# haan6/fm-for-online-recommendation

Measured on AMD Instinct MI355X. Metric: samples/sec online-FM (Criteo-39-field, k=16) FTRL-proximal, higher is better.
Workload: dtype f32

## Files before the change

fm-for-online-recommendation_amd/csrc/fmx_common.h:

```cpp
#pragma once
#include <hip/hip_runtime.h>
#include <hip/hip_ext.h>

#include <cstdarg>
#include <cstdio>
#include <cstdlib>
#include <cstring>
#include <atomic>
#include <mutex>

#include "fmx.h"

#pragma clang fp contract(off)

namespace fmxd {
extern thread_local char g_err[512];
int fail(int code, const char *fmt, ...);
int check_launch(const char *what);

struct Tune {
  int wpb_fwd = 4, wpb_upd = 2;
  int sort_e = 0;
  int inline_fixup = 1;
  int online_persistent = 1;
// ... 202 lines not shown
    s = s + xor_lane_f4<M>(s, lane);
    ss = ss + xor_lane_f4<M>(ss, lane);
    fo += xor_lane_f<M>(fo, lane);
  }
}
template <int LPR>
__device__ __forceinline__ void fm_field_sums(float4 &s, float4 &ss, float &fo, int lane, int groups = WAVE) {
  fm_sums_level<1, LPR>(s, ss, fo, lane, groups);
  fm_sums_level<2, LPR>(s, ss, fo, lane, groups);
  fm_sums_level<4, LPR>(s, ss, fo, lane, groups);
  fm_sums_level<8, LPR>(s, ss, fo, lane, groups);
  fm_sums_level<16, LPR>(s, ss, fo, lane, groups);
  fm_sums_level<32, LPR>(s, ss, fo, lane, groups);
}
template <int LPR>
__device__ __forceinline__ float4 fm_bi(float4 s, float4 ss, float &sbi) {
  const float4 bi = 0.5f * (s * s - ss);
  sbi = (bi.x + bi.y) + (bi.z + bi.w);
#pragma unroll
  for (int m = 1; m < LPR; m <<= 1) sbi += __shfl_xor(sbi, m);
  return bi;
}
template <int LPR>
__device__ __forceinline__ float4 fm_bi_dpp(float4 s, float4 ss, float &sbi) {
  const float4 bi = 0.5f * (s * s - ss);
  sbi = (bi.x + bi.y) + (bi.z + bi.w);
  if (LPR > 1) sbi += xor_lane_f<1>(sbi, 0);
  if (LPR > 2) sbi += xor_lane_f<2>(sbi, 0);
  if (LPR > 4) sbi += xor_lane_f<4>(sbi, 0);
  if (LPR > 8) sbi += xor_lane_f<8>(sbi, 0);
  return bi;
}

__device__ float block_sum(const float *src, int n, int ld, float *sm) {
  constexpr int U = 16;
  const int tid = threadIdx.x, nt = blockDim.x < 128 ? blockDim.x : 128;
  float acc = 0.f;
  if (tid >= nt) {
    __syncthreads();
    for (int w = nt >> 1; w > 0; w >>= 1) __syncthreads();
    const float r = sm[0];
    __syncthreads();
    return r;
  }
  if (ld == 1) {
    const int n4 = n >> 2;
    const float4 *src4 = reinterpret_cast<const float4 *>(src);
    for (int i0 = tid; i0 < n4; i0 += U * nt) {
      float4 v[U];
#pragma unroll
      for (int u = 0; u < U; ++u) {
        const int i = i0 + u * nt;
        v[u] = src4[i < n4 ? i : 0];
      }
#pragma unroll
      for (int u = 0; u < U; ++u) {
        const bool in = i0 + u * nt < n4;
        acc += in ? (v[u].x + v[u].y) + (v[u].z + v[u].w) : 0.f;
      }
    }
    for (int i = (n4 << 2) + tid; i < n; i += nt) acc += src[i];
  } else {
    constexpr int V = 4;
    const int n4 = n >> 2;
    for (int i0 = tid; i0 < n4; i0 += V * nt) {
      float4 v[V];
#pragma unroll
      for (int u = 0; u < V; ++u) {
        const int i = i0 + u * nt;
        const float *p = src + (size_t)(4 * (i < n4 ? i : 0)) * ld;
        v[u] = float4{p[0], p[ld], p[2 * (size_t)ld], p[3 * (size_t)ld]};
      }
#pragma unroll
      for (int u = 0; u < V; ++u) {
        const bool in = i0 + u * nt < n4;
        acc += in ? (v[u].x + v[u].y) + (v[u].z + v[u].w) : 0.f;
      }
    }
    for (int i = (n4 << 2) + tid; i < n; i += nt) acc += src[(size_t)i * ld];
  }
  sm[tid] = acc;
  __syncthreads();
  for (int w = nt >> 1; w > 0; w >>= 1) {
    if (tid < w) sm[tid] += sm[tid + w];
    __syncthreads();
  }
  const float r = sm[0];
  __syncthreads();
  return r;
}

__device__ __forceinline__ float ld_sc1(const float *p) {
  return __hip_atomic_load(p, __ATOMIC_RELAXED, __HIP_MEMORY_SCOPE_AGENT);
}
__device__ __forceinline__ float4 ld_sc1_4(const float *p) { return {ld_sc1(p), ld_sc1(p + 1), ld_sc1(p + 2), ld_sc1(p + 3)}; }

__device__ __forceinline__ void st16(float *p, float4 v) {
  typedef float f4v __attribute__((ext_vector_type(4)));
  __builtin_nontemporal_store(f4v{v.x, v.y, v.z, v.w}, reinterpret_cast<f4v *>(p));
}
__device__ __forceinline__ void st4(float *p, float v) { __builtin_nontemporal_store(v, p); }

struct RowRegs {
  float4 v;
  float4 z, n;
  float4 fo;
};

template <int LAYOUT, int RULE>
__device__ __forceinline__ RowRegs load_row(const float *rp, int q, int kp, int zoff) {
  RowRegs r;
  r.v = *reinterpret_cast<const float4 *>(rp + 4 * q);
  r.z = splat(0.f);
  r.n = splat(0.f);
  r.fo = splat(0.f);
  if (LAYOUT == FMX_LAYOUT_WEIGHTS) {
    r.fo.x = rp[kp];
  } else {
    if (LAYOUT == FMX_LAYOUT_FTRL || RULE == FMX_RULE_ADAM) r.z = *reinterpret_cast<const float4 *>(rp + zoff + 4 * q);
    r.n = *reinterpret_cast<const float4 *>(rp + zoff + kp + 4 * q);
    r.fo = *reinterpret_cast<const float4 *>(rp + kp);
  }
  return r;
}

template <int LAYOUT, int RULE>
__device__ __forceinline__ void update_row(float *rp, int q, int kp, int zoff, RowRegs r, float4 cV, float4 cA, float cw,
                                           const fmx_hyper_t &h) {
// ... 142 lines not shown
```

fm-for-online-recommendation_amd/csrc/fmx_kernels.hip:

```cpp

#include <type_traits>

#include "fmx_common.h"

namespace fmxd {

thread_local char g_err[512] = "";

int fail(int code, const char *fmt, ...) {
  va_list ap;
  va_start(ap, fmt);
  vsnprintf(g_err, sizeof(g_err), fmt, ap);
  va_end(ap);
  return code;
}

int check_launch(const char *what) {
  hipError_t e = hipGetLastError();
  if (e != hipSuccess) return fail(FMX_ERR_LAUNCH, "%s: %s", what, hipGetErrorString(e));
  return FMX_OK;
}

}

// ... 356 lines not shown
      bce_loss_dz(a.loss_kind, z, y_early, a.inv_b, loss, dz);
      if (a.out.loss) a.out.loss[(size_t)b * a.ld1] = loss;
      if (a.out.dz) a.out.dz[(size_t)b * a.ld1] = dz;
    }
  }
}

struct UpdArgs {
  float *rows;
  const int64_t *foff;
  float *bias;
  const uint32_t *sorted;
  float *parts;
  int32_t *meta;
  const float *xv;
  const float *S;
  const float *dz_first;
  const float *dz_bi;
  const float *gbi;
  const float *loss_b;
  float *loss_out;
  int32_t *step_counter;
  fmx_hyper_t h;
  int32_t B, F, Bp, bbits, kp, stride, zoff;
  int32_t ldS, ld1;
  int32_t ldG;
  const int32_t *cols;
  const int32_t *fcols;
  int32_t Fx;
  float *red;
  uint32_t seq;
  int32_t *error;
  float inv_b;
};

constexpr int LEAD_NONE = 0, LEAD_CLOSES = 1, LEAD_THROUGH = 2;

constexpr int RED_SLICE = 4096;
__host__ __device__ inline int red_slices(int B) { return (B + RED_SLICE - 1) / RED_SLICE; }

template <int LAYOUT, int RULE>
__device__ __forceinline__ void apply_bias_and_loss(const UpdArgs &a, float db, float ls) {
  constexpr bool MOM = LAYOUT == FMX_LAYOUT_MOMENTS;
  float b0 = a.bias[0], b1 = LAYOUT != FMX_LAYOUT_WEIGHTS ? a.bias[1] : 0.f, b2 = MOM ? a.bias[2] : 0.f;
  bias_step<LAYOUT, RULE>(b0, b1, b2, db, a.h);
  st4(a.bias, b0);
  if (LAYOUT == FMX_LAYOUT_FTRL || (MOM && RULE == FMX_RULE_ADAM)) st4(a.bias + 1, b1);
  if (MOM) st4(a.bias + 2, b2);
  if (a.loss_b && a.loss_out) {
    int i = 0;
    if (a.step_counter) {
      i = *a.step_counter;
      *a.step_counter = i + 1;
    }
    a.loss_out[i] = ls * a.inv_b;
  }
}

template <int LAYOUT, int RULE>
__device__ void finish_bias_and_loss(const UpdArgs &a, int R, bool poll) {
  __shared__ float part[2 * 16];
  const int t = threadIdx.x;
  bool failed = false;
  if (t < R) {
    const v4f *src = reinterpret_cast<const v4f *>(a.red) + t;
    v4f g = {0.f, 0.f, 0.f, 0.f};
    if (poll) {
      for (int spin = 0;; ++spin) {
        asm volatile("global_load_dwordx4 %0, %1, off sc1\n\ts_waitcnt vmcnt(0)" : "=v"(g) : "v"(src) : "memory");
        if (__float_as_uint(g.z) == a.seq) break;
        if (spin >= (1 << 20)) {
          failed = true;
          break;
        }
        __builtin_amdgcn_s_sleep(1);
      }
    } else {
      g = *src;
    }
    part[2 * t] = g.x;
    part[2 * t + 1] = g.y;
  }
  if (failed && a.error) *a.error = 2;
  __syncthreads();
  if (t == 0) {
    float db = 0.f, ls = 0.f;
    for (int r = 0; r < R; ++r) {
      db += part[2 * r];
      ls += part[2 * r + 1];
    }
    apply_bias_and_loss<LAYOUT, RULE>(a, db, ls);
  }
}

template <int LAYOUT, int RULE, bool INL>
__device__ void bias_and_loss(const UpdArgs &a, int r) {
  __shared__ float sm[256];
  const int R = red_slices(a.B);
  const int first = r * RED_SLICE, n = (a.B - first) < RED_SLICE ? (a.B - first) : RED_SLICE;
  const float db = block_sum(a.dz_first + (size_t)first * a.ld1, n, a.ld1, sm);
  float ls = 0.f;
  if (a.loss_b && a.loss_out) ls = block_sum(a.loss_b + (size_t)first * a.ld1, n, a.ld1, sm);
  if (R == 1) {
    if (threadIdx.x == 0) apply_bias_and_loss<LAYOUT, RULE>(a, db, ls);
    return;
  }
  if (threadIdx.x == 0) st_sc1_4(a.red + 4 * r, float4{db, ls, __uint_as_float(a.seq), 0.f});
  if (INL && r == 0) finish_bias_and_loss<LAYOUT, RULE>(a, R, true);
}

__device__ __forceinline__ void store_part(float *rec, int q, int kp, float4 cV, float4 cA, float cw) {
  *reinterpret_cast<float4 *>(rec + 4 * q) = cV;
  *reinterpret_cast<float4 *>(rec + kp + 4 * q) = cA;
  if (q == 0) rec[2 * kp] = cw;
}

template <bool VEC> struct CoefA;
template <> struct CoefA<true> {
  float4 v;
  __device__ __forceinline__ void zero() { v = splat(0.f); }
  __device__ __forceinline__ void add(const CoefA &o) { v = v + o.v; }
  __device__ __forceinline__ float4 vec() const { return v; }
  __device__ __forceinline__ CoefA up(int d) const { return {shfl_up4(v, d)}; }
};
template <> struct CoefA<false> {
  float v;
  __device__ __forceinline__ void zero() { v = 0.f; }
  __device__ __forceinline__ void add(const CoefA &o) { v += o.v; }
  __device__ __forceinline__ float4 vec() const { return splat(v); }
  __device__ __forceinline__ CoefA up(int d) const { return {__shfl_up(v, d)}; }
};

#ifdef FMX_STAMPS
__device__ unsigned long long g_upd_stamps[8192 * 6];
#define FMX_STAMP(slot_, dep_)                                                                                      \
  do {                                                                                                              \
    unsigned long long t_;                                                                                          \
    asm volatile("s_memrealtime %0\n\ts_waitcnt lgkmcnt(0)" : "=s"(t_) : "v"(dep_) : "memory");                      \
    if (lane == 0 && gt < 8192) g_upd_stamps[(size_t)gt * 6 + (slot_)] = t_;                                         \
  } while (0)
#else
#define FMX_STAMP(slot_, dep_) do {} while (0)
#endif

template <int LPR, int LAYOUT, int RULE, bool HAS_GBI, bool INL, bool OCC = false>
__device__ __forceinline__ void update_body(const UpdArgs &a, const int blk) {
  constexpr int SLOTS = WAVE / LPR;
  constexpr int EPG = LPR;
  constexpr int REC = 2 * LPR * 4 + 4;
  constexpr bool PREFETCH_ROWS = EPG <= 4;
  using CA = CoefA<HAS_GBI>;
  const int n_red = red_slices(a.B);
  if (blk < n_red) {
    bias_and_loss<LAYOUT, RULE, INL>(a, blk);
    return;
  }
  const int lane = threadIdx.x & 63;
  const int slot = lane / LPR, q = lane % LPR;
  const int kp = LPR * 4;
  const int tiles_per_field = a.Bp >> 6;
  const int gt = (blk - n_red) * (blockDim.x >> 6) + (threadIdx.x >> 6);
  if (gt >= a.F * tiles_per_field) return;
  const int f = gt / tiles_per_field;
  const int base = (gt - f * tiles_per_field) << 6;
  const uint32_t *sf = a.sorted + (size_t)f * a.Bp;
  const int bbits = a.bbits;
  const uint32_t bmask = (1u << bbits) - 1u;
  const int e0 = base + slot * EPG;
  FMX_STAMP(0, lane);

  uint32_t c[EPG];
  if constexpr (EPG % 4 == 0) {
#pragma unroll
    for (int j = 0; j < EPG; j += 4) {
      const uint4 t = *reinterpret_cast<const uint4 *>(sf + e0 + j);
      c[j] = t.x;
      c[j + 1] = t.y;
      c[j + 2] = t.z;
      c[j + 3] = t.w;
    }
  } else {
#pragma unroll
    for (int j = 0; j < EPG; ++j) c[j] = sf[e0 + j];
  }
  const uint32_t kprev = (e0 == 0 ? SENT : sf[e0 - 1]) >> bbits;
  const uint32_t knext = (e0 + EPG < a.Bp ? sf[e0 + EPG] : SENT) >> bbits;
  const uint32_t tile_prevkey = (base == 0 ? SENT : sf[base - 1]) >> bbits;
// ... 26 lines not shown
    if (INL)
      row_in = load_row<LAYOUT, RULE>(a.rows + (row0 + ((slot == 0 && run_comes_in) ? tile_prevkey : 0u)) * (size_t)a.stride, q, kp, a.zoff);
  };
  const bool tile_open_early = INL && __shfl((int)(val[EPG - 1] && k[EPG - 1] == knext), WAVE - 1) != 0;
  float4 cV[EPG];
  CA cA[EPG];
  float cw[EPG];
  {
    const bool has_x = a.xv != nullptr;
    const float *xsrc = has_x ? a.xv : a.dz_first;
    const int fld = (has_x && a.cols) ? a.cols[f] : f;
    const int col = (has_x && a.fcols) ? a.fcols[fld] : fld;
    int efld = 0;
    if constexpr (OCC) efld = a.cols ? a.cols[f] : f;
    float4 S4[EPG], G4[EPG];
    float xl[EPG], dzf[EPG], dzbl[EPG];
    uint32_t bj[EPG];
#pragma unroll
    for (int j = 0; j < EPG; ++j) bj[j] = val[j] ? (c[j] & bmask) : 0u;
    const bool sep_dzbi = a.dz_bi != nullptr && a.dz_bi != a.dz_first;
#pragma unroll
    for (int j = 0; j < EPG; ++j) {
      xl[j] = 1.f;
      dzbl[j] = 0.f;
    }
    if (has_x) {
#pragma unroll
      for (int j = 0; j < EPG; ++j) xl[j] = xsrc[(size_t)bj[j] * a.Fx + col];
    }
    if (sep_dzbi) {
#pragma unroll
      for (int j = 0; j < EPG; ++j) dzbl[j] = a.dz_bi[(size_t)bj[j] * a.ld1];
    }
#pragma unroll
    for (int j = 0; j < EPG; ++j) {
      const uint32_t b = bj[j];
      if constexpr (OCC) S4[j] = *reinterpret_cast<const float4 *>(a.gbi + (size_t)b * a.ldG + (size_t)efld * kp + 4 * q);
      else S4[j] = *reinterpret_cast<const float4 *>(a.S + (size_t)b * a.ldS + 4 * q);
      dzf[j] = a.dz_first[(size_t)b * a.ld1];
      if constexpr (HAS_GBI) G4[j] = *reinterpret_cast<const float4 *>(a.gbi + (size_t)b * a.ldG + 4 * q);
      else G4[j] = splat(0.f);
    }
    if (!tile_open_early) request_rows();
#pragma unroll
    for (int j = 0; j < EPG; ++j) {
      const float x = xl[j];
      const float dzb = a.dz_bi ? (sep_dzbi ? dzbl[j] : dzf[j]) : 0.f;
      const float w1 = x * dzf[j];
      float4 v;
      CA ca;
      if constexpr (OCC) {
        v = S4[j];
        ca.zero();
      } else if constexpr (HAS_GBI) {
        const float4 G = splat(dzb) + G4[j];
        const float4 xG = x * G;
        v = xG * S4[j];
        ca.v = x * xG;
      } else {
        const float xG = x * dzb;
        v = xG * S4[j];
        ca.v = x * xG;
      }
      cV[j] = splat(0.f);
      cA[j].zero();
      cw[j] = 0.f;
      if (val[j]) {
        cV[j] = v;
        cA[j] = ca;
        cw[j] = w1;
      }
    }
  }

  float4 tV = splat(0.f);
  CA tA;
// ... 137 lines not shown
      }
      __builtin_amdgcn_s_sleep(1);
    }
  }
  if (failed || m == 0 || m > t) {
    if (lane == 0 && a.error) *a.error = 2;
    return;
  }
  const size_t gh = (size_t)gt - m;
  float4 aV = splat(0.f), aA = splat(0.f);
  float aw = 0.f;
  for (int j = slot; j <= m; j += SLOTS) {
    if (j == m) {
      aV = aV + ownV;
      aA = aA + ownA;
      aw += ownw;
    } else {
      const float *rec = j == 0 ? a.parts + (gh * 2 + 1) * REC : a.parts + (gh + j) * 2 * REC;
      aV = aV + ld_sc1_4(rec + 4 * q);
      aA = aA + ld_sc1_4(rec + kp + 4 * q);
      aw += ld_sc1(rec + 2 * kp);
    }
  }
#pragma unroll
  for (int mm = LPR; mm < WAVE; mm <<= 1) {
    aV = aV + shfl_xor4(aV, mm);
    aA = aA + shfl_xor4(aA, mm);
    aw += __shfl_xor(aw, mm);
  }
  if (lane < LPR) update_row<LAYOUT, RULE>(rp, q, kp, a.zoff, r, aV, aA, aw, a.h);
  FMX_STAMP(4, lane);
}

template <int LPR, int LAYOUT, int RULE, bool HAS_GBI, bool INL>
__global__ __launch_bounds__(256) void k_fm_update(UpdArgs a) {
  __builtin_amdgcn_s_setprio(3);
  update_body<LPR, LAYOUT, RULE, HAS_GBI, INL>(a, blockIdx.x);
}

template <int LPR, int LAYOUT, int RULE, bool INL>
__global__ __launch_bounds__(256) void k_fm_update_occ(UpdArgs a) {
  __builtin_amdgcn_s_setprio(3);
  update_body<LPR, LAYOUT, RULE, false, INL, true>(a, blockIdx.x);
}

template <int LPR, int LAYOUT, int RULE, bool HAS_GBI>
__global__ __launch_bounds__(256) void k_fm_update_rider(UpdArgs a, MlpReduceArgs r, int n_update_blocks, int rider_blocks_per_layer) {
  __builtin_amdgcn_s_setprio(3);
  if ((int)blockIdx.x >= n_update_blocks) {
    const int rb = (int)blockIdx.x - n_update_blocks;
    mlp_reduce_block(r, rb / rider_blocks_per_layer, rb % rider_blocks_per_layer, rider_blocks_per_layer);
    return;
  }
  update_body<LPR, LAYOUT, RULE, HAS_GBI, true>(a, blockIdx.x);
}

struct OnlineArgs {
  float *rows;
  const int64_t *foff;
  float *bias;
  const int32_t *idx;
  const float *xv;
  const float *y;
  uint8_t *pred;
  float *loss;
  int32_t *error;
  fmx_hyper_t h;
  int32_t N, F, stride, zoff, loss_kind;
};

// ... 703 lines not shown
  snprintf(msg, sizeof(msg), "%s", g_err);
  return fail(rc, "%s: %s", who, msg);
}
Tune &tune() {
  static Tune t = [] {
    Tune x;
    if (const char *e = getenv("FMX_WPB_FWD")) x.wpb_fwd = atoi(e);
    if (const char *e = getenv("FMX_WPB_UPD")) x.wpb_upd = atoi(e);
    if (const char *e = getenv("FMX_SORT_E")) x.sort_e = atoi(e);
    if (const char *e = getenv("FMX_SORT_AHEAD")) x.sort_ahead = atoi(e);
    if (const char *e = getenv("FMX_ONLINE_PERSISTENT")) x.online_persistent = atoi(e);
    if (const char *e = getenv("FMX_INLINE_FIXUP")) x.inline_fixup = atoi(e);
    if (const char *e = getenv("FMX_SORT_CHUNKED")) x.sort_chunked = atoi(e);
    if (const char *e = getenv("FMX_MLP_CHAIN")) x.mlp_chain = atoi(e);
    auto ok = [](int v) { return v == 1 || v == 2 || v == 4; };
    if (!ok(x.wpb_fwd)) x.wpb_fwd = 4;
    if (!ok(x.wpb_upd)) x.wpb_upd = 2;
    return x;
  }();
  return t;
}
}
namespace {

constexpr int SORT_AHEAD_MAX = 16;

struct Workspace {
  uint32_t *sorted;
  size_t sorted_stride;
  uint32_t *runs;
  int32_t *meta;
  int32_t *counter;
  float *parts;
  size_t bytes;
};



Workspace carve(const fmx_table_t *t, int B, void *base) {
  const size_t F = (size_t)n_sort_fields(t), Bp = (size_t)fmx_sorted_width(B), tiles = Bp >> 6;
  const size_t rec = 2 * (size_t)t->kp + 4;
  const size_t o_sorted1 = align_up(F * Bp * 4, 256);
  const size_t o_runs = 2 * SORT_AHEAD_MAX * o_sorted1;
  const size_t o_meta = o_runs + (Bp >= 2 * SORT_CHUNK ? SORT_AHEAD_MAX * o_sorted1 : 0);
  const size_t o_counter = o_meta + align_up(F * tiles * 2 * 4, 256);
  const size_t o_parts = o_counter + 256;
  Workspace w;
  char *p = static_cast<char *>(base);
  w.sorted = reinterpret_cast<uint32_t *>(p);
  w.sorted_stride = o_sorted1 / 4;
  w.runs = reinterpret_cast<uint32_t *>(p + o_runs);
  w.meta = reinterpret_cast<int32_t *>(p + o_meta);
  w.counter = reinterpret_cast<int32_t *>(p + o_counter);
  w.parts = reinterpret_cast<float *>(p + o_parts);
  w.bytes = o_parts + align_up(F * tiles * 2 * rec * 4, 256);
  return w;
}

int check_workspace(const fmx_table_t *t, int B, const void *workspace, int64_t workspace_bytes, const char *who) {
  if (!workspace) return fail(FMX_ERR_ARG, "%s: null workspace", who);
  if (!aligned16(workspace)) return fail(FMX_ERR_ALIGN, "%s: workspace must be 16-byte aligned", who);
  const int64_t need = (int64_t)carve(t, B, nullptr).bytes;
  if (workspace_bytes < need)
    return fail(FMX_ERR_SHAPE, "%s: workspace of %lld bytes, %lld needed for B = %d and %d sort fields (fmx_workspace_bytes)", who,
                (long long)workspace_bytes, (long long)need, B, n_sort_fields(t));
  return FMX_OK;
}

struct Side {
  hipStream_t stream = nullptr;
  hipStream_t main = nullptr;
  hipEvent_t fork = nullptr, sorted[2] = {nullptr, nullptr}, consumed[2] = {nullptr, nullptr};
  hipEvent_t user_fork = nullptr, user_join = nullptr;
};

Side *side_for_current_device() {
  static std::mutex mu;
  static Side sides[64];
  int dev = 0;
  if (hipGetDevice(&dev) != hipSuccess || dev < 0 || dev >= 64) return nullptr;
  std::lock_guard<std::mutex> lock(mu);
  Side &sd = sides[dev];
  if (!sd.stream) {
    int lo = 0, hi = 0;
    (void)hipDeviceGetStreamPriorityRange(&lo, &hi);
    if (hipStreamCreateWithPriority(&sd.stream, hipStreamNonBlocking, lo) != hipSuccess) return nullptr;
    if (hipStreamCreateWithPriority(&sd.main, hipStreamNonBlocking, hi) != hipSuccess) return nullptr;
    bool ok = hipEventCreateWithFlags(&sd.fork, hipEventDisableTiming) == hipSuccess &&
// ... 4 lines not shown
           hipEventCreateWithFlags(&sd.consumed[i], hipEventDisableTiming) == hipSuccess;
    }
    if (!ok) return nullptr;
  }
  return &sd;
}

constexpr int OVERLAP_MIN_BATCH = 512;

template <int LPR, int NPASS, bool MAPPED = false>
void launch_forward_np(const FwdArgs &a, int layout, hipStream_t st) {
  const int wpb = tune().wpb_fwd;
  const dim3 grid((a.B + wpb - 1) / wpb), block(64 * wpb);
  if (layout == FMX_LAYOUT_FTRL) hipLaunchKernelGGL((k_fm_forward<LPR, FMX_LAYOUT_FTRL, NPASS, MAPPED>), grid, block, 0, st, a);
  else hipLaunchKernelGGL((k_fm_forward<LPR, FMX_LAYOUT_WEIGHTS, NPASS, MAPPED>), grid, block, 0, st, a);
}

template <int LPR>
void launch_forward(const FwdArgs &a, int layout, hipStream_t st) {
  const int slots = WAVE / LPR;
  const int np = (a.F + slots - 1) / slots;
  if (a.fcols || a.fbase)
    launch_forward_np<LPR, 0, true>(a, layout, st);
  else if (!with_one_of<1, 2, 3, 4>(np, [&](auto NP) { launch_forward_np<LPR, NP>(a, layout, st); }))
    launch_forward_np<LPR, 0>(a, layout, st);
}

bool is_capturing(hipStream_t st) {
  if (!st) return false;
  hipStreamCaptureStatus cs = hipStreamCaptureStatusNone;
  return hipStreamIsCapturing(st, &cs) == hipSuccess && cs != hipStreamCaptureStatusNone;
}

template <int LPR, bool HAS_GBI, bool INL>
void launch_update(const UpdArgs &a, int rule, hipStream_t st) {
  const int tiles = a.F * (a.Bp >> 6);
  const int wpb = tune().wpb_upd;
  const dim3 grid((tiles + wpb - 1) / wpb + red_slices(a.B)), block(64 * wpb);
  with_rule(rule, [&](auto LAYOUT, auto RULE) { hipLaunchKernelGGL((k_fm_update<LPR, LAYOUT, RULE, HAS_GBI, INL>), grid, block, 0, st, a); });
}

template <int LPR>
void launch_update_rider(const UpdArgs &a, int rule, const MlpReduceArgs &r, hipStream_t st) {
  const int tiles = a.F * (a.Bp >> 6);
  const int wpb = tune().wpb_upd;
  const int n_upd = (tiles + wpb - 1) / wpb + red_slices(a.B), per = mlp_reduce_blocks_per_layer(r, 64 * wpb);
  const dim3 grid(n_upd + per * r.n_layers), block(64 * wpb);
  with_rule(rule, [&](auto LAYOUT, auto RULE) {
    hipLaunchKernelGGL((k_fm_update_rider<LPR, LAYOUT, RULE, true>), grid, block, 0, st, a, r, n_upd, per);
  });
}

template <int LPR>
void launch_fixup(const UpdArgs &a, int rule, hipStream_t st) {
  const int tiles = a.F * (a.Bp >> 6);
  const int wpb = tune().wpb_upd;
  const dim3 grid((tiles + wpb - 1) / wpb + (red_slices(a.B) > 1 ? 1 : 0)), block(64 * wpb);
  with_rule(rule, [&](auto LAYOUT, auto RULE) { hipLaunchKernelGGL((k_fm_fixup<LPR, LAYOUT, RULE>), grid, block, 0, st, a); });
}

template <int LPR>
void launch_update_pair(const UpdArgs &a, int rule, bool has_gbi, hipStream_t st) {
  if (tune().inline_fixup && !is_capturing(st)) {
    if (has_gbi) launch_update<LPR, true, true>(a, rule, st);
    else launch_update<LPR, false, true>(a, rule, st);
    return;
  }
  if (has_gbi) launch_update<LPR, true, false>(a, rule, st);
  else launch_update<LPR, false, false>(a, rule, st);
  launch_fixup<LPR>(a, rule, st);
}

template <int LPR>
void launch_update_occ_pair(const UpdArgs &a, int rule, hipStream_t st) {
  const int tiles = a.F * (a.Bp >> 6);
  const int wpb = tune().wpb_upd;
  const dim3 grid((tiles + wpb - 1) / wpb + red_slices(a.B)), block(64 * wpb);
  const bool inl = tune().inline_fixup && !is_capturing(st);
  with_rule(rule, [&](auto LAYOUT, auto RULE) {
    if (inl) hipLaunchKernelGGL((k_fm_update_occ<LPR, LAYOUT, RULE, true>), grid, block, 0, st, a);
    else hipLaunchKernelGGL((k_fm_update_occ<LPR, LAYOUT, RULE, false>), grid, block, 0, st, a);
  });
  if (!inl) launch_fixup<LPR>(a, rule, st);
}

template <int E>
void launch_sort(SortArgs a, hipStream_t st) {
  const int threads = a.Bp / E;
  uint32_t lds = (uint32_t)(a.Bp * sizeof(uint32_t));
  if (a.Bp <= RADIX_SMALL_WIDTH && threads >= 64) {
    a.small_bits = RADIX_SMALL_BITS;
    const uint32_t need = (uint32_t)radix_small_lds_bytes(a.Bp, threads);
    if (need > lds) lds = need;
  }
  const int grid = a.n_batches >= 8 ? 8 * a.F * ((a.n_batches + 7) / 8) : a.F * a.n_batches;
  hipLaunchKernelGGL((k_sort_occ<E>), dim3(grid), dim3(threads), lds, st, a);
}

int prepare_sort(int B) {
  if ((size_t)fmx_sorted_width(B) * 4 <= 64 * 1024) return FMX_OK;
  static std::mutex mu;
// ... 210 lines not shown
  a.ldG = sample_ld > 0 ? sample_ld : table->kp;
  static std::atomic<uint32_t> launch_seq{1};
  a.seq = launch_seq.fetch_add(1) & 0x0FFFFFFFu;
  if (a.seq == 0) a.seq = launch_seq.fetch_add(1) & 0x0FFFFFFFu;
  a.error = err_flag;
  a.rows = table->rows;
  a.foff = sort_offsets(table);
  a.cols = sort_cols(table);
  a.Fx = n_cols(table);
  a.fcols = table->field_cols;
  a.bias = table->bias;
  a.sorted = sorted;
  a.parts = w.parts;
  a.meta = w.meta;
  a.red = reinterpret_cast<float *>(w.counter);
  a.xv = xv;
  a.S = S;
  a.dz_first = dz_first;
  a.dz_bi = dz_bi;
  a.gbi = gbi;
  a.loss_b = loss_b;
  a.loss_out = loss_out;
  a.step_counter = step_counter;
  a.h = hyper_for(hyper, -1);
  a.B = B;
  a.F = n_sort_fields(table);
  a.Bp = fmx_sorted_width(B);
  a.bbits = fmx_sorted_bbits(B);
  a.kp = table->kp;
  a.stride = table->row_stride;
  a.zoff = table->z_offset;
  a.h.alpha = 1.0f / hyper->alpha;
  a.inv_b = inv_b;
  return a;
}

int update_impl(const fmx_table_t *table, const fmx_hyper_t *hyper, int32_t rule, const Workspace &w,
                const uint32_t *sorted, const float *xv,
                const float *S, const float *dz_first, const float *dz_bi, const float *gbi, int32_t B,
                const float *loss_b, float inv_b, float *loss_out, hipStream_t st,
                int32_t *step_counter = nullptr, int32_t sample_ld = 0,
                int32_t *err_flag = nullptr, const MlpReduceArgs *rider = nullptr) {
  UpdArgs a = fill_upd(table, hyper, w, sorted, xv, S, dz_first, dz_bi, gbi, B, loss_b, inv_b, loss_out, step_counter,
                       sample_ld, err_flag);
  if (rule == FMX_RULE_ADAM)
    adam_consts(hyper->lr, hyper->beta1, hyper->beta2, hyper->step + 1, a.h.lr, a.h.beta1, a.h.beta2);
  if (rider) {
    if (gbi != nullptr && tune().inline_fixup && !is_capturing(st)) {
      with_lpr(table->kp, [&](auto LPR) { launch_update_rider<LPR>(a, rule, *rider, st); });
      return check_launch("k_fm_update_rider");
    }
    mlp_launch_reduce(*rider, st);
  }
  with_lpr(table->kp, [&](auto LPR) { launch_update_pair<LPR>(a, rule, gbi != nullptr, st); });
  return check_launch("k_fm_update / k_fm_fixup");
}

int update_occ_impl(const fmx_table_t *table, const fmx_hyper_t *hyper, int32_t rule, const Workspace &w, const float *xv,
                    const float *dz_first, const float *occ, int32_t ld_occ, int32_t B, const float *loss_b, float inv_b,
                    float *loss_out, hipStream_t st) {
  UpdArgs a = fill_upd(table, hyper, w, w.sorted, xv, nullptr, dz_first, nullptr, occ, B, loss_b, inv_b, loss_out, nullptr, 0,
                       nullptr);
  a.ldG = ld_occ;
  if (rule == FMX_RULE_ADAM) adam_consts(hyper->lr, hyper->beta1, hyper->beta2, hyper->step + 1, a.h.lr, a.h.beta1, a.h.beta2);
  with_lpr(table->kp, [&](auto LPR) { launch_update_occ_pair<LPR>(a, rule, st); });
  return check_launch("k_fm_update_occ / k_fm_fixup");
}

template <int LPR, int LAYOUT, int RULE>
void launch_online_np(const OnlineArgs &a, int np, hipStream_t st) {
  auto launch = [&](auto NP) { hipLaunchKernelGGL((k_fm_online<LPR, LAYOUT, RULE, NP>), dim3(1), dim3(64), 0, st, a); };
  if (!with_one_of<1, 2, 3>(np, launch)) launch(std::integral_constant<int, 4>{});
}

constexpr int ONLINE_MLP_MAX_PARAMS = 8192;
constexpr int ONLINE_MLP_OPT_MAX_PARAMS = 8192;

// ... 362 lines not shown
  (void)hipStreamWaitEvent(st, c->ready[slot], 0);
  if (int rc = part_impl(table, idx_all, nullptr, GB, c->n_blocks, c->block_count[c->rank], B, bufs->parts_send, error, st)) return rc;
  if (int rc = comm_exchange_blocks(c, bufs->parts_send, bufs->parts_recv, (size_t)B * rec_in, st)) return rc;
  fmx_fwd_out_t out;
  memset(&out, 0, sizeof(out));
  out.S = bufs->rec_local;
  out.dz = bufs->rec_local + kp;
  out.loss = bufs->rec_local + kp + 1;
  out.sample_ld = rec_out;
  out.error = error;
  if (int rc = fmx_fm_forward_finish(hyper, table->bias, table->layout, kp, bufs->parts_recv, (int64_t)B * rec_in, c->n_blocks, y_local, B,
                                     loss_kind, inv_b, &out, stream))
    return rc;
  if (int rc = comm_all_gather(c, 0, bufs->rec_local, bufs->rec_all, (size_t)B * rec_out, st)) return rc;
  const Workspace w = carve(table, GB, workspace);
  const float *rec = bufs->rec_all;
  if (int rc = update_impl(table, hyper, rule, w, w.sorted, nullptr, rec, rec + kp, rec + kp, nullptr, GB, rec + kp + 1, inv_b, loss_out, st,
                           nullptr, rec_out, error))
    return rc;
  (void)hipEventRecord(c->free_[slot], st);
  c->used[slot] = true;
  return FMX_OK;
}

int fmx_fm_step(const fmx_table_t *table, const fmx_hyper_t *hyper, int32_t rule, int32_t loss_kind,
                const int32_t *idx, const float *xv, const float *y, int32_t B, float inv_b, void *workspace, int64_t workspace_bytes,
                const fmx_fwd_out_t *fwd, float *loss_out, fmx_stream_t stream) {
  if (int rc = check_step_args(table, hyper, rule, loss_kind, B, workspace, fwd)) return rc;
  if (!idx || !y) return fail(FMX_ERR_ARG, "fmx_fm_step: idx and y are required");
  hipStream_t st = static_cast<hipStream_t>(stream);
  if (int rc = check_workspace(table, B, workspace, workspace_bytes, "fmx_fm_step")) return rc;
  const Workspace w = carve(table, B, workspace);
  if (int rc = sort_impl(table, idx, B, w.sorted, w.runs, fwd->error, st)) return rc;
  if (int rc = forward_impl(table, hyper, idx, xv, y, B, loss_kind, inv_b, fwd, st)) return rc;
  return update_impl(table, hyper, rule, w, w.sorted, xv, fwd->S, fwd->dz, fwd->dz, nullptr, B, fwd->loss, inv_b, loss_out, st,
                     nullptr, fwd->sample_ld, fwd->error);
}

int fmx_fm_stream(const fmx_table_t *table, const fmx_hyper_t *hyper, int32_t rule, int32_t loss_kind,
                  const int32_t *idx_pool, const float *y_pool, int32_t n_pool, int32_t B, float inv_b,
                  int32_t n_steps, void *workspace, int64_t workspace_bytes, const fmx_fwd_out_t *fwd, float *loss_out, float *kernel_ms,
                  fmx_stream_t stream) {
  if (int rc = check_step_args(table, hyper, rule, loss_kind, B, workspace, fwd)) return rc;
  if (!idx_pool || !y_pool || n_pool < 1 || n_steps < 0) return fail(FMX_ERR_ARG, "fmx_fm_stream: bad pool / step count");
  if (int rc = check_adam(hyper, rule, n_steps)) return rc;
  hipStream_t st = static_cast<hipStream_t>(stream);
  if (int rc = check_workspace(table, B, workspace, workspace_bytes, "fmx_fm_stream")) return rc;
  const Workspace w = carve(table, B, workspace);
  if (!kernel_ms) {
    auto forward = [&](int, const int32_t *idx, const float *y, hipStream_t st) {
      return forward_impl(table, hyper, idx, nullptr, y, B, loss_kind, inv_b, fwd, st);
    };
    auto update = [&](int s, const uint32_t *sorted, hipStream_t st) {
      fmx_hyper_t hs = hyper_for(hyper, rule);
      hs.step += s;
      return update_impl(table, &hs, rule, w, sorted, nullptr, fwd->S, fwd->dz, fwd->dz, nullptr, B, fwd->loss, inv_b,
                         loss_out ? loss_out + s : nullptr, st, nullptr, fwd->sample_ld, fwd->error);
    };
    return pool_loop(table, idx_pool, y_pool, n_pool, B, n_steps, w, fwd->error, st, forward, update);
  }

  const int REP = 8, n_ev = 5;
  const int n_groups = (n_steps + REP - 1) / REP;
  const size_t F = (size_t)n_cols(table);
  const size_t region = align_up((size_t)B * table->kp + 2 * (size_t)B, 64);
  float *tmp = nullptr;
  hipEvent_t *ev = nullptr;
  int rc = FMX_OK;
  {
    const Detour detour(st == nullptr ? side_for_current_device() : nullptr, st);
    st = detour.st;
    if (n_groups > 0 && hipMalloc(&tmp, REP * region * sizeof(float)) != hipSuccess)
      return fail(FMX_ERR_LAUNCH, "hipMalloc (measuring mode)");
    ev = new hipEvent_t[(size_t)n_groups * n_ev];
    for (int i = 0; i < n_groups * n_ev; ++i) (void)hipEventCreate(&ev[i]);
    for (int g = 0; g < n_groups && rc == FMX_OK; ++g) {
      const int first = g * REP, n = (n_steps - first) < REP ? (n_steps - first) : REP;
      hipEvent_t *e = ev + (size_t)g * n_ev;
      (void)hipEventRecord(e[0], st);
      rc = sort_pool(table, idx_pool, n_pool, B, first, n, w, w.sorted, fwd->error, st);
      (void)hipEventRecord(e[1], st);
      for (int r = 0; r < n && rc == FMX_OK; ++r) {
        const int j = (first + r) % n_pool;
        fmx_fwd_out_t fr = *fwd;
        fr.S = tmp + (size_t)r * region;
        fr.dz = fr.S + (size_t)B * table->kp;
        fr.loss = fr.dz + B;
        fr.sample_ld = 0;
        rc = forward_impl(table, hyper, idx_pool + (size_t)j * B * F, nullptr, y_pool + (size_t)j * B, B, loss_kind, inv_b, &fr, st);
      }
      (void)hipEventRecord(e[2], st);
      for (int r = 0; r < n && rc == FMX_OK; ++r) {
        const float *S = tmp + (size_t)r * region, *dz = S + (size_t)B * table->kp;
        fmx_hyper_t hs = hyper_for(hyper, rule);
        hs.step += first + r;
        rc = update_impl(table, &hs, rule, w, w.sorted + (size_t)r * w.sorted_stride, nullptr, S, dz, dz, nullptr, B, dz + B, inv_b,
                         loss_out ? loss_out + first + r : nullptr, st, nullptr, 0, fwd->error);
      }
      (void)hipEventRecord(e[3], st);
      (void)hipEventRecord(e[4], st);
    }
    (void)hipStreamSynchronize(st);
  }
  for (int k = 0; k < 4; ++k) kernel_ms[k] = 0.f;
  if (rc == FMX_OK && n_groups > 0) {
    double t_sort = 0, t_fwd = 0, t_upd = 0, t_pair = 0;
    for (int g = 0; g < n_groups; ++g) {
      hipEvent_t *e = ev + (size_t)g * n_ev;
      float pair = 0.f, ms[3] = {0.f, 0.f, 0.f};
      (void)hipEventElapsedTime(&pair, e[3], e[4]);
      for (int k = 0; k < 3; ++k) (void)hipEventElapsedTime(&ms[k], e[k], e[k + 1]);
      t_pair += pair;
      t_sort += fmaxf(ms[0] - pair, 0.f);
      t_fwd += fmaxf(ms[1] - pair, 0.f);
      t_upd += fmaxf(ms[2] - pair, 0.f);
    }
    kernel_ms[0] = (float)(t_sort / n_groups * n_steps);
    kernel_ms[1] = (float)t_fwd;
    kernel_ms[2] = (float)t_upd;
    kernel_ms[3] = (float)(t_pair / n_groups * n_steps);
  }
  for (int i = 0; i < n_groups * n_ev; ++i) (void)hipEventDestroy(ev[i]);
  delete[] ev;
  if (tmp) (void)hipFree(tmp);
  return rc;
}

int fmx_fm_online_run(const fmx_table_t *table, const fmx_hyper_t *hyper, int32_t rule, int32_t loss_kind,
                      const int32_t *idx, const float *xv, const float *y, int32_t N, uint8_t *pred_out, float *loss_out,
                      int32_t *error, fmx_stream_t stream) {
// ... 324 lines not shown
```

Before: 199.7 million.

## Evaluate BCE loss and dlogit inside the FM update kernel instead of forward

The forward pass now writes only logits (loss kind NONE), and the update kernel recomputes loss and dz from logit and label. Update lanes compute dz for their own samples while row loads are in flight. Extra lead blocks write dz and loss for the bias and loss reduction, using per-slice flags and a spin-wait to coordinate. This moves loss evaluation off the forward critical path and overlaps it with the update's memory waits. The cost is more update work, extra lead blocks, spin synchronisation, and a larger workspace carve.

```diff
diff --git a/fm-for-online-recommendation_amd/csrc/fmx_common.h b/fm-for-online-recommendation_amd/csrc/fmx_common.h
--- a/fm-for-online-recommendation_amd/csrc/fmx_common.h
+++ b/fm-for-online-recommendation_amd/csrc/fmx_common.h
@@ -258,6 +258,15 @@
   return bi;
 }
 
+__device__ __forceinline__ float ld_sc1(const float *p) {
+  return __hip_atomic_load(p, __ATOMIC_RELAXED, __HIP_MEMORY_SCOPE_AGENT);
+}
+__device__ __forceinline__ float4 ld_sc1_4(const float *p) { return {ld_sc1(p), ld_sc1(p + 1), ld_sc1(p + 2), ld_sc1(p + 3)}; }
+template <bool SC1>
+__device__ __forceinline__ float blk_ld(const float *p) { return SC1 ? ld_sc1(p) : *p; }
+template <bool SC1>
+__device__ __forceinline__ float4 blk_ld4(const float *p) { return SC1 ? ld_sc1_4(p) : *reinterpret_cast<const float4 *>(p); }
+template <bool SC1 = false>
 __device__ float block_sum(const float *src, int n, int ld, float *sm) {
   constexpr int U = 16;
   const int tid = threadIdx.x, nt = blockDim.x < 128 ? blockDim.x : 128;
@@ -271,13 +280,12 @@
   }
   if (ld == 1) {
     const int n4 = n >> 2;
-    const float4 *src4 = reinterpret_cast<const float4 *>(src);
     for (int i0 = tid; i0 < n4; i0 += U * nt) {
       float4 v[U];
 #pragma unroll
       for (int u = 0; u < U; ++u) {
         const int i = i0 + u * nt;
-        v[u] = src4[i < n4 ? i : 0];
+        v[u] = blk_ld4<SC1>(src + 4 * (size_t)(i < n4 ? i : 0));
       }
 #pragma unroll
       for (int u = 0; u < U; ++u) {
@@ -285,7 +293,7 @@
         acc += in ? (v[u].x + v[u].y) + (v[u].z + v[u].w) : 0.f;
       }
     }
-    for (int i = (n4 << 2) + tid; i < n; i += nt) acc += src[i];
+    for (int i = (n4 << 2) + tid; i < n; i += nt) acc += blk_ld<SC1>(src + i);
   } else {
     constexpr int V = 4;
     const int n4 = n >> 2;
@@ -295,7 +303,7 @@
       for (int u = 0; u < V; ++u) {
         const int i = i0 + u * nt;
         const float *p = src + (size_t)(4 * (i < n4 ? i : 0)) * ld;
-        v[u] = float4{p[0], p[ld], p[2 * (size_t)ld], p[3 * (size_t)ld]};
+        v[u] = float4{blk_ld<SC1>(p), blk_ld<SC1>(p + ld), blk_ld<SC1>(p + 2 * (size_t)ld), blk_ld<SC1>(p + 3 * (size_t)ld)};
       }
 #pragma unroll
       for (int u = 0; u < V; ++u) {
@@ -303,7 +311,7 @@
         acc += in ? (v[u].x + v[u].y) + (v[u].z + v[u].w) : 0.f;
       }
     }
-    for (int i = (n4 << 2) + tid; i < n; i += nt) acc += src[(size_t)i * ld];
+    for (int i = (n4 << 2) + tid; i < n; i += nt) acc += blk_ld<SC1>(src + (size_t)i * ld);
   }
   sm[tid] = acc;
   __syncthreads();
@@ -316,10 +324,6 @@
   return r;
 }
 
-__device__ __forceinline__ float ld_sc1(const float *p) {
-  return __hip_atomic_load(p, __ATOMIC_RELAXED, __HIP_MEMORY_SCOPE_AGENT);
-}
-__device__ __forceinline__ float4 ld_sc1_4(const float *p) { return {ld_sc1(p), ld_sc1(p + 1), ld_sc1(p + 2), ld_sc1(p + 3)}; }
 
 __device__ __forceinline__ void st16(float *p, float4 v) {
   typedef float f4v __attribute__((ext_vector_type(4)));
diff --git a/fm-for-online-recommendation_amd/csrc/fmx_kernels.hip b/fm-for-online-recommendation_amd/csrc/fmx_kernels.hip
--- a/fm-for-online-recommendation_amd/csrc/fmx_kernels.hip
+++ b/fm-for-online-recommendation_amd/csrc/fmx_kernels.hip
@@ -412,6 +412,10 @@
   uint32_t seq;
   int32_t *error;
   float inv_b;
+  const float *logit, *y;
+  float *dz_w, *loss_w;
+  int32_t *eflags;
+  int32_t loss_kind;
 };
 
 constexpr int LEAD_NONE = 0, LEAD_CLOSES = 1, LEAD_THROUGH = 2;
@@ -473,14 +477,83 @@
   }
 }
 
-template <int LAYOUT, int RULE, bool INL>
-__device__ void bias_and_loss(const UpdArgs &a, int r) {
+constexpr int RED_EVAL = 8;
+#ifdef FMX_STAMPS
+__device__ unsigned long long g_upd_stamps[8192 * 6];
+#define FMX_LEAD_STAMP(blk_, slot_)                                                                                 \
+  do {                                                                                                              \
+    unsigned long long t_;                                                                                          \
+    asm volatile("s_memrealtime %0\n\ts_waitcnt lgkmcnt(0)" : "=s"(t_) : : "memory");                               \
+    if (threadIdx.x == 0 && (blk_) < 64) g_upd_stamps[(size_t)(8191 - (blk_)) * 6 + (slot_)] = t_;                    \
+  } while (0)
+#else
+#define FMX_LEAD_STAMP(blk_, slot_) do {} while (0)
+#endif
+template <bool INL, bool EVAL>
+__host__ __device__ inline int lead_blocks(int B) { return red_slices(B) * (EVAL && INL ? RED_EVAL : 1); }
+
+template <bool INL>
+__device__ __forceinline__ bool eval_slice(const UpdArgs &a, int r, int h) {
+  constexpr int E = INL ? RED_EVAL : 1, U = 4;
+  const int first = r * RED_SLICE, n = (a.B - first) < RED_SLICE ? (a.B - first) : RED_SLICE;
+  const int t = threadIdx.x, step = E * blockDim.x;
+  const float *zs = a.logit + first, *ys = a.y + first;
+  float *dzw = a.dz_w + (size_t)first * a.ld1, *lsw = a.loss_w + (size_t)first * a.ld1;
+  for (int e0 = h * blockDim.x + t; e0 < n; e0 += U * step) {
+    float z[U], y[U];
+#pragma unroll
+    for (int u = 0; u < U; ++u) {
+      const int e = e0 + u * step;
+      z[u] = zs[e < n ? e : 0];
+      y[u] = ys[e < n ? e : 0];
+    }
+#pragma unroll
+    for (int u = 0; u < U; ++u) {
+      const int e = e0 + u * step;
+      float loss, dz;
+      bce_loss_dz(a.loss_kind, z[u], y[u], a.inv_b, loss, dz);
+      if (e < n) {
+        st_sc1(dzw + (size_t)e * a.ld1, dz);
+        st_sc1(lsw + (size_t)e * a.ld1, loss);
+      }
+    }
+  }
+  asm volatile("s_waitcnt vmcnt(0)" ::: "memory");
+  __syncthreads();
+  if (E == 1) return true;
+  int32_t *flags = a.eflags + r * RED_EVAL;
+  if (t == 0) __hip_atomic_store(flags + h, (int32_t)a.seq, __ATOMIC_RELAXED, __HIP_MEMORY_SCOPE_AGENT);
+  if (h != 0) return false;
+  if (t < E) {
+    bool failed = false;
+    for (int spin = 0;; ++spin) {
+      if (__hip_atomic_load(flags + t, __ATOMIC_RELAXED, __HIP_MEMORY_SCOPE_AGENT) == (int32_t)a.seq) break;
+      if (spin >= (1 << 20)) {
+        failed = true;
+        break;
+      }
+      __builtin_amdgcn_s_sleep(1);
+    }
+    if (failed && a.error) *a.error = 2;
+  }
+  __syncthreads();
+  return true;
+}
+
+template <int LAYOUT, int RULE, bool INL, bool EVAL>
+__device__ void bias_and_loss(const UpdArgs &a, int blk) {
   __shared__ float sm[256];
   const int R = red_slices(a.B);
+  int r = blk;
+  if constexpr (EVAL) {
+    constexpr int E = INL ? RED_EVAL : 1;
+    r = blk / E;
+    if (!eval_slice<INL>(a, r, blk - r * E)) return;
+  }
   const int first = r * RED_SLICE, n = (a.B - first) < RED_SLICE ? (a.B - first) : RED_SLICE;
-  const float db = block_sum(a.dz_first + (size_t)first * a.ld1, n, a.ld1, sm);
+  const float db = block_sum<EVAL>(a.dz_first + (size_t)first * a.ld1, n, a.ld1, sm);
   float ls = 0.f;
-  if (a.loss_b && a.loss_out) ls = block_sum(a.loss_b + (size_t)first * a.ld1, n, a.ld1, sm);
+  if (a.loss_b && a.loss_out) ls = block_sum<EVAL>(a.loss_b + (size_t)first * a.ld1, n, a.ld1, sm);
   if (R == 1) {
     if (threadIdx.x == 0) apply_bias_and_loss<LAYOUT, RULE>(a, db, ls);
     return;
@@ -512,7 +585,6 @@
 };
 
 #ifdef FMX_STAMPS
-__device__ unsigned long long g_upd_stamps[8192 * 6];
 #define FMX_STAMP(slot_, dep_)                                                                                      \
   do {                                                                                                              \
     unsigned long long t_;                                                                                          \
@@ -523,16 +595,37 @@
 #define FMX_STAMP(slot_, dep_) do {} while (0)
 #endif
 
-template <int LPR, int LAYOUT, int RULE, bool HAS_GBI, bool INL, bool OCC = false>
+template <int LPR, int J>
+__device__ __forceinline__ float group_lane_f(float v, int lane) {
+  if constexpr (LPR == 1) {
+    return v;
+  } else if constexpr (LPR == 2) {
+    return __int_as_float(__builtin_amdgcn_mov_dpp(__float_as_int(v), J ? 0xF5 : 0xA0, 0xF, 0xF, true));
+  } else if constexpr (LPR == 4) {
+    return __int_as_float(__builtin_amdgcn_mov_dpp(__float_as_int(v), J * 0x55, 0xF, 0xF, true));
+  } else {
+    return __shfl(v, (lane & ~(LPR - 1)) + J);
+  }
+}
+template <int LPR, int J = 0>
+__device__ __forceinline__ void group_lanes_f(float (&dst)[LPR], float v, int lane) {
+  dst[J] = group_lane_f<LPR, J>(v, lane);
+  if constexpr (J + 1 < LPR) group_lanes_f<LPR, J + 1>(dst, v, lane);
+}
+
+template <int LPR, int LAYOUT, int RULE, bool HAS_GBI, bool INL, bool OCC = false, bool EVAL = false>
 __device__ __forceinline__ void update_body(const UpdArgs &a, const int blk) {
+  static_assert(!EVAL || (!HAS_GBI && !OCC), "dlogit is evaluated in the update for the pure FM only");
   constexpr int SLOTS = WAVE / LPR;
   constexpr int EPG = LPR;
   constexpr int REC = 2 * LPR * 4 + 4;
   constexpr bool PREFETCH_ROWS = EPG <= 4;
   using CA = CoefA<HAS_GBI>;
-  const int n_red = red_slices(a.B);
+  const int n_red = lead_blocks<INL, EVAL>(a.B);
   if (blk < n_red) {
-    bias_and_loss<LAYOUT, RULE, INL>(a, blk);
+    FMX_LEAD_STAMP(blk, 0);
+    bias_and_loss<LAYOUT, RULE, INL, EVAL>(a, blk);
+    FMX_LEAD_STAMP(blk, 1);
     return;
   }
   const int lane = threadIdx.x & 63;
@@ -625,16 +718,42 @@
 #pragma unroll
       for (int j = 0; j < EPG; ++j) dzbl[j] = a.dz_bi[(size_t)bj[j] * a.ld1];
     }
+    float zq = 0.f, yq = 0.f;
+    if constexpr (EVAL) {
+      uint32_t bq = bj[0];
+#pragma unroll
+      for (int j = 1; j < EPG; ++j) bq = q == j ? bj[j] : bq;
+      zq = a.logit[bq];
+      yq = a.y[bq];
+    }
 #pragma unroll
     for (int j = 0; j < EPG; ++j) {
       const uint32_t b = bj[j];
       if constexpr (OCC) S4[j] = *reinterpret_cast<const float4 *>(a.gbi + (size_t)b * a.ldG + (size_t)efld * kp + 4 * q);
       else S4[j] = *reinterpret_cast<const float4 *>(a.S + (size_t)b * a.ldS + 4 * q);
-      dzf[j] = a.dz_first[(size_t)b * a.ld1];
+      if constexpr (!EVAL) dzf[j] = a.dz_first[(size_t)b * a.ld1];
       if constexpr (HAS_GBI) G4[j] = *reinterpret_cast<const float4 *>(a.gbi + (size_t)b * a.ldG + 4 * q);
       else G4[j] = splat(0.f);
     }
-    if (!tile_open_early) request_rows();
+    if constexpr (EVAL) {
+      auto eval_dz = [&]() {
+        float lq, dq;
+        bce_loss_dz(a.loss_kind, zq, yq, a.inv_b, lq, dq);
+        group_lanes_f<LPR>(dzf, dq, lane);
+      };
+      if (!tile_open_early) {
+        request_rows();
+        eval_dz();
+#pragma unroll
+        for (int j = 0; j < EPG; ++j) asm volatile("; dlogit under the row wait" : "+v"(dzf[j]));
+      } else {
+        eval_dz();
+#pragma unroll
+        for (int j = 0; j < EPG; ++j) asm volatile("; dlogit ahead of the publication" : "+v"(dzf[j]));
+      }
+    } else {
+      if (!tile_open_early) request_rows();
+    }
 #pragma unroll
     for (int j = 0; j < EPG; ++j) {
       const float x = xl[j];
@@ -838,10 +957,10 @@
   FMX_STAMP(4, lane);
 }
 
-template <int LPR, int LAYOUT, int RULE, bool HAS_GBI, bool INL>
+template <int LPR, int LAYOUT, int RULE, bool HAS_GBI, bool INL, bool EVAL = false>
 __global__ __launch_bounds__(256) void k_fm_update(UpdArgs a) {
   __builtin_amdgcn_s_setprio(3);
-  update_body<LPR, LAYOUT, RULE, HAS_GBI, INL>(a, blockIdx.x);
+  update_body<LPR, LAYOUT, RULE, HAS_GBI, INL, false, EVAL>(a, blockIdx.x);
 }
 
 template <int LPR, int LAYOUT, int RULE, bool INL>
@@ -1611,6 +1730,8 @@
   int32_t *meta;
   int32_t *counter;
   float *parts;
+  int32_t *eflags;
+  float *logit;
   size_t bytes;
 };
 
@@ -1632,7 +1753,11 @@
   w.meta = reinterpret_cast<int32_t *>(p + o_meta);
   w.counter = reinterpret_cast<int32_t *>(p + o_counter);
   w.parts = reinterpret_cast<float *>(p + o_parts);
-  w.bytes = o_parts + align_up(F * tiles * 2 * rec * 4, 256);
+  const size_t o_eflags = o_parts + align_up(F * tiles * 2 * rec * 4, 256);
+  const size_t o_logit = o_eflags + align_up(16 * RED_EVAL * 4, 256);
+  w.eflags = reinterpret_cast<int32_t *>(p + o_eflags);
+  w.logit = reinterpret_cast<float *>(p + o_logit);
+  w.bytes = o_logit + align_up((size_t)B * 4, 256);
   return w;
 }
 
@@ -1703,12 +1828,14 @@
   return hipStreamIsCapturing(st, &cs) == hipSuccess && cs != hipStreamCaptureStatusNone;
 }
 
-template <int LPR, bool HAS_GBI, bool INL>
+template <int LPR, bool HAS_GBI, bool INL, bool EVAL = false>
 void launch_update(const UpdArgs &a, int rule, hipStream_t st) {
   const int tiles = a.F * (a.Bp >> 6);
   const int wpb = tune().wpb_upd;
-  const dim3 grid((tiles + wpb - 1) / wpb + red_slices(a.B)), block(64 * wpb);
-  with_rule(rule, [&](auto LAYOUT, auto RULE) { hipLaunchKernelGGL((k_fm_update<LPR, LAYOUT, RULE, HAS_GBI, INL>), grid, block, 0, st, a); });
+  const dim3 grid((tiles + wpb - 1) / wpb + lead_blocks<INL, EVAL>(a.B)), block(64 * wpb);
+  with_rule(rule, [&](auto LAYOUT, auto RULE) {
+    hipLaunchKernelGGL((k_fm_update<LPR, LAYOUT, RULE, HAS_GBI, INL, EVAL>), grid, block, 0, st, a);
+  });
 }
 
 template <int LPR>
@@ -1732,12 +1859,15 @@
 
 template <int LPR>
 void launch_update_pair(const UpdArgs &a, int rule, bool has_gbi, hipStream_t st) {
+  const bool eval = a.logit != nullptr;
   if (tune().inline_fixup && !is_capturing(st)) {
     if (has_gbi) launch_update<LPR, true, true>(a, rule, st);
+    else if (eval) launch_update<LPR, false, true, true>(a, rule, st);
     else launch_update<LPR, false, true>(a, rule, st);
     return;
   }
   if (has_gbi) launch_update<LPR, true, false>(a, rule, st);
+  else if (eval) launch_update<LPR, false, false, true>(a, rule, st);
   else launch_update<LPR, false, false>(a, rule, st);
   launch_fixup<LPR>(a, rule, st);
 }
@@ -2014,7 +2144,21 @@
   a.zoff = table->z_offset;
   a.h.alpha = 1.0f / hyper->alpha;
   a.inv_b = inv_b;
+  a.logit = a.y = nullptr;
+  a.dz_w = a.loss_w = nullptr;
+  a.eflags = w.eflags;
+  a.loss_kind = FMX_LOSS_NONE;
   return a;
+}
+
+struct StepEval {
+  const float *logit, *y;
+  int32_t loss_kind;
+};
+fmx_fwd_out_t step_forward_out(const fmx_fwd_out_t *fwd, const Workspace &w) {
+  fmx_fwd_out_t o = *fwd;
+  if (!o.logit) o.logit = w.logit;
+  return o;
 }
 
 int update_impl(const fmx_table_t *table, const fmx_hyper_t *hyper, int32_t rule, const Workspace &w,
@@ -2022,9 +2166,16 @@
                 const float *S, const float *dz_first, const float *dz_bi, const float *gbi, int32_t B,
                 const float *loss_b, float inv_b, float *loss_out, hipStream_t st,
                 int32_t *step_counter = nullptr, int32_t sample_ld = 0,
-                int32_t *err_flag = nullptr, const MlpReduceArgs *rider = nullptr) {
+                int32_t *err_flag = nullptr, const MlpReduceArgs *rider = nullptr, const StepEval *eval = nullptr) {
   UpdArgs a = fill_upd(table, hyper, w, sorted, xv, S, dz_first, dz_bi, gbi, B, loss_b, inv_b, loss_out, step_counter,
                        sample_ld, err_flag);
+  if (eval) {
+    a.logit = eval->logit;
+    a.y = eval->y;
+    a.loss_kind = eval->loss_kind;
+    a.dz_w = const_cast<float *>(dz_first);
+    a.loss_w = const_cast<float *>(loss_b);
+  }
   if (rule == FMX_RULE_ADAM)
     adam_consts(hyper->lr, hyper->beta1, hyper->beta2, hyper->step + 1, a.h.lr, a.h.beta1, a.h.beta2);
   if (rider) {
@@ -2453,9 +2604,11 @@
   if (int rc = check_workspace(table, B, workspace, workspace_bytes, "fmx_fm_step")) return rc;
   const Workspace w = carve(table, B, workspace);
   if (int rc = sort_impl(table, idx, B, w.sorted, w.runs, fwd->error, st)) return rc;
-  if (int rc = forward_impl(table, hyper, idx, xv, y, B, loss_kind, inv_b, fwd, st)) return rc;
+  const fmx_fwd_out_t fo = step_forward_out(fwd, w);
+  if (int rc = forward_impl(table, hyper, idx, xv, y, B, FMX_LOSS_NONE, inv_b, &fo, st)) return rc;
+  const StepEval ev{fo.logit, y, loss_kind};
   return update_impl(table, hyper, rule, w, w.sorted, xv, fwd->S, fwd->dz, fwd->dz, nullptr, B, fwd->loss, inv_b, loss_out, st,
-                     nullptr, fwd->sample_ld, fwd->error);
+                     nullptr, fwd->sample_ld, fwd->error, nullptr, &ev);
 }
 
 int fmx_fm_stream(const fmx_table_t *table, const fmx_hyper_t *hyper, int32_t rule, int32_t loss_kind,
@@ -2469,14 +2622,16 @@
   if (int rc = check_workspace(table, B, workspace, workspace_bytes, "fmx_fm_stream")) return rc;
   const Workspace w = carve(table, B, workspace);
   if (!kernel_ms) {
+    const fmx_fwd_out_t fo = step_forward_out(fwd, w);
     auto forward = [&](int, const int32_t *idx, const float *y, hipStream_t st) {
-      return forward_impl(table, hyper, idx, nullptr, y, B, loss_kind, inv_b, fwd, st);
+      return forward_impl(table, hyper, idx, nullptr, y, B, FMX_LOSS_NONE, inv_b, &fo, st);
     };
     auto update = [&](int s, const uint32_t *sorted, hipStream_t st) {
       fmx_hyper_t hs = hyper_for(hyper, rule);
       hs.step += s;
+      const StepEval ev{fo.logit, y_pool + (size_t)(s % n_pool) * B, loss_kind};
       return update_impl(table, &hs, rule, w, sorted, nullptr, fwd->S, fwd->dz, fwd->dz, nullptr, B, fwd->loss, inv_b,
-                         loss_out ? loss_out + s : nullptr, st, nullptr, fwd->sample_ld, fwd->error);
+                         loss_out ? loss_out + s : nullptr, st, nullptr, fwd->sample_ld, fwd->error, nullptr, &ev);
     };
     return pool_loop(table, idx_pool, y_pool, n_pool, B, n_steps, w, fwd->error, st, forward, update);
   }
@@ -2484,7 +2639,7 @@
   const int REP = 8, n_ev = 5;
   const int n_groups = (n_steps + REP - 1) / REP;
   const size_t F = (size_t)n_cols(table);
-  const size_t region = align_up((size_t)B * table->kp + 2 * (size_t)B, 64);
+  const size_t region = align_up((size_t)B * table->kp + 3 * (size_t)B, 64);
   float *tmp = nullptr;
   hipEvent_t *ev = nullptr;
   int rc = FMX_OK;
@@ -2507,16 +2662,18 @@
         fr.S = tmp + (size_t)r * region;
         fr.dz = fr.S + (size_t)B * table->kp;
         fr.loss = fr.dz + B;
+        fr.logit = fr.loss + B;
         fr.sample_ld = 0;
-        rc = forward_impl(table, hyper, idx_pool + (size_t)j * B * F, nullptr, y_pool + (size_t)j * B, B, loss_kind, inv_b, &fr, st);
+        rc = forward_impl(table, hyper, idx_pool + (size_t)j * B * F, nullptr, y_pool + (size_t)j * B, B, FMX_LOSS_NONE, inv_b, &fr, st);
       }
       (void)hipEventRecord(e[2], st);
       for (int r = 0; r < n && rc == FMX_OK; ++r) {
         const float *S = tmp + (size_t)r * region, *dz = S + (size_t)B * table->kp;
         fmx_hyper_t hs = hyper_for(hyper, rule);
         hs.step += first + r;
+        const StepEval ev{dz + 2 * (size_t)B, y_pool + (size_t)((first + r) % n_pool) * B, loss_kind};
         rc = update_impl(table, &hs, rule, w, w.sorted + (size_t)r * w.sorted_stride, nullptr, S, dz, dz, nullptr, B, dz + B, inv_b,
-                         loss_out ? loss_out + first + r : nullptr, st, nullptr, 0, fwd->error);
+                         loss_out ? loss_out + first + r : nullptr, st, nullptr, 0, fwd->error, nullptr, &ev);
       }
       (void)hipEventRecord(e[3], st);
       (void)hipEventRecord(e[4], st);
```

New measurement: 191.1 million. 0.957x the previous value.
